# wicstas/pine

Measured on AMD Instinct MI355X. Metric: Msamples/s, higher is better.
Workload: dtype f32

## Files before the change

include/pine_gpu.h:

```cpp
#ifndef PINE_GPU_H
#define PINE_GPU_H
#include <stddef.h>
#include <stdint.h>
#ifdef __cplusplus
extern "C" {
#endif

#define PINE_GPU_ABI_VERSION 4

typedef struct pine_gpu_scene pine_gpu_scene;
typedef struct pine_gpu_plan pine_gpu_plan;

const char* pine_gpu_last_error(void);
float pine_gpu_progress(void);
int pine_gpu_abi_version(void);

void pine_gpu_mat4_identity(float out[16]);
void pine_gpu_mat4_translate(const float v[3], float out[16]);
void pine_gpu_mat4_scale(const float v[3], float out[16]);
void pine_gpu_mat4_rotate_x(float rad, float out[16]);
void pine_gpu_mat4_rotate_y(float rad, float out[16]);
void pine_gpu_mat4_rotate_z(float rad, float out[16]);
void pine_gpu_mat4_mul(const float a[16], const float b[16], float out[16]);
void pine_gpu_mat4_inverse(const float m[16], float out[16]);
// ... 145 lines not shown
  int32_t samples_per_item;
  int32_t grid_blocks;
  int32_t block_threads;
  int32_t lds_bytes;
  int32_t timed_launches;
  uint64_t walk_steps;
  float accel_build_ms;
  float upload_ms;
  int32_t accel_built_on_device;
  int32_t serial_tiles;
  int32_t specialized;
  float specialize_ms;
  uint32_t kernel_features;
  int32_t specialize_source;
  int32_t specialize_pending;
  int32_t reserved;
} pine_gpu_plan_stats;
int64_t pine_gpu_scene_specialized_source(pine_gpu_scene*, char* out, int64_t cap);
int pine_gpu_test_specialize_compile(pine_gpu_scene*, uint32_t features, int ctx, const char* arch, char* path_out, int64_t cap);
int pine_gpu_scene_build_accel_device(pine_gpu_scene*, int device);
int pine_gpu_plan_stats_get(pine_gpu_plan*, pine_gpu_plan_stats* out);
int pine_gpu_plan_check(pine_gpu_plan*);

int pine_gpu_plan_debug_sections(pine_gpu_plan*, uint64_t out[16]);
int64_t pine_gpu_plan_vertex_log(pine_gpu_plan*, float* out, int64_t capacity_floats);

int pine_gpu_plan_read_samples(pine_gpu_plan*, float* out_host, int64_t capacity_floats);

pine_gpu_plan* pine_gpu_plan_create_passes(pine_gpu_scene*, const pine_gpu_render_params*, int32_t pass_samples);
int pine_gpu_plan_pass_count(pine_gpu_plan*);
int pine_gpu_plan_pass_info(pine_gpu_plan*, int pass, int32_t out[4]);
// ... 65 lines not shown
```

pine_amd/_lib.py:

```python
import ctypes as C
import os

_HERE = os.path.dirname(os.path.abspath(__file__))
LIB_PATH = os.environ.get("PINE_GPU_LIB") or os.path.join(_HERE, "lib", "libpine_gpu.so")
TABLE_PATH = os.path.join(_HERE, "data", "bluesobol_u8.bin")

if not os.path.exists(LIB_PATH):
    raise ImportError(
        f"{LIB_PATH} not found: build the HIP extension first (python -c 'import __graft_entry__ as g; g.build()' "
        "or make -C pine_amd/csrc). pine_amd has no CPU fallback."
    )
lib = C.CDLL(LIB_PATH)

f3 = C.c_float * 3
f16 = C.c_float * 16
c_f_p = C.POINTER(C.c_float)


class RenderParams(C.Structure):
    _fields_ = [
        ("spp", C.c_int32),
        ("max_path_length", C.c_int32),
        ("device", C.c_int32),
        ("shard_rank", C.c_int32),
# ... 16 lines not shown
        ("samples_per_item", C.c_int32),
        ("grid_blocks", C.c_int32),
        ("block_threads", C.c_int32),
        ("lds_bytes", C.c_int32),
        ("timed_launches", C.c_int32),
        ("walk_steps", C.c_uint64),
        ("accel_build_ms", C.c_float),
        ("upload_ms", C.c_float),
        ("accel_built_on_device", C.c_int32),
        ("serial_tiles", C.c_int32),
        ("specialized", C.c_int32),
        ("specialize_ms", C.c_float),
        ("kernel_features", C.c_uint32),
        ("specialize_source", C.c_int32),
        ("specialize_pending", C.c_int32),
        ("reserved", C.c_int32),
    ]


FLAG_TIMING = 1
FLAG_PROGRESS = 2
FLAG_FAST = 4
FLAG_DEVICE_BVH = 8
FLAG_DEBUG_FORCE_BAIL = 0x100
FLAG_VERTEX_LOG = 0x200
FLAG_SPECIALIZE = 0x400
FLAG_SPECIALIZE_NO_BAKE = 0x800
FLAG_SPECIALIZE_ASYNC = 0x1000
FLAG_NO_SPECIALIZE = 0x2000
FLAG_ORDER_EMBREE = 0x4000
FLAG_ORDER_NEAREST = FLAG_ORDER_EMBREE
# ... 148 lines not shown
```

pine_amd/csrc/pine_kernels.hip:

```cpp
#include <hip/hip_runtime.h>

#include <climits>
#include <cmath>
#include <cstring>
#include <deque>

#include "pine_plan.h"
#include "pine_bvh_build_device.h"
#include "pine_embree_order.h"
#include "../data/rcpps_table.h"
namespace pine_gpu {

static int device_build(std::vector<BuildPrim>& prims, const std::vector<BuildTask>& roots, FlatAccel& A, int device) {
  int ndev = 0;
  if (hipGetDeviceCount(&ndev) != hipSuccess || device < 0 || device >= ndev) {
    (void)hipGetLastError();
    return -1;
  }
  if (hipSetDevice(device) != hipSuccess) return -1;
  const size_t n = prims.size();
  BuildPrim *d_prims = nullptr, *d_scratch = nullptr;
  BuildTask *d_tasks[2] = {nullptr, nullptr};
  BuildDecision* d_dec = nullptr;
  int *d_rank = nullptr, *d_perm = nullptr, *d_src = nullptr, *d_counts = nullptr;
// ... 63 lines not shown
    }
    auto by_order = [](const PineKernelVariant& a, const PineKernelVariant& b) { return a.order < b.order; };
    std::sort(queue.begin(), queue.end(), by_order);
    std::sort(mega.begin(), mega.end(), by_order);
  }
};
static const VariantTables& variant_tables() {
  static const VariantTables t;
  return t;
}
#define kVariants (variant_tables().mega)
#define kQueueVariants (variant_tables().queue)
#define kNumVariants (int(variant_tables().mega.size()))
#define kNumQueueVariants (int(variant_tables().queue.size()))

struct ResolvePass {
  int film_w, film_h, spp;
  int whole_tiles, slice_first, slice_tiles;
  int free_rows;
  int first_pass;
  int samples_so_far;
  int packed;
};
__global__ void __launch_bounds__(kBlock) resolve_kernel(WorkParams W, ResolvePass R, const float4* __restrict__ samples,
                                                        float4* __restrict__ sum, float4* __restrict__ film,
                                                        Counters* __restrict__ counters) {
  const unsigned long long t = blockIdx.x * (unsigned long long)kBlock + threadIdx.x;
  const int ltile = int(t >> 6);
  if (ltile >= W.num_local_tiles) return;
  const int p = int(t & 63);
  const int tile = film_tile_of(W, ltile);
  const int px = (tile % W.tiles_x) * kTile + (p & 7), py = (tile / W.tiles_x) * kTile + (p >> 3);
  const bool inside = px < R.film_w && py < R.film_h;
  const float4* row = nullptr;
  int rows = 0;
  bool carried = false, shown = true;
  float divisor = float(R.spp);
  if (ltile < R.whole_tiles) {
    if (ltile >= R.slice_first && ltile < R.slice_first + R.slice_tiles) {
      row = samples + (unsigned long long)(ltile - R.slice_first) * (unsigned)R.spp * 64ull + p;
      rows = R.spp;
    } else if (ltile < R.slice_first) {
      carried = true;
    } else {
      shown = false;
    }
  } else {
    row = samples + ((unsigned long long)R.slice_tiles * (unsigned)R.spp + (unsigned long long)(ltile - R.whole_tiles) * (unsigned)R.free_rows) * 64ull + p;
    rows = R.free_rows;
    carried = !R.first_pass;
    divisor = float(R.samples_so_far);
  }
  if (!inside) rows = 0;
  float4* const acc = sum && inside ? sum + (unsigned long long)ltile * 64ull + p : nullptr;
  f3 L = mk3(0.0f);
  if (carried && acc) {
    const float4 a = *acc;
    L = f3{a.x, a.y, a.z};
  }
  unsigned long long verts = 0;
  int s = 0;
  for (; s + 8 <= rows; s += 8) {
    float4 v[8];
#pragma unroll
    for (int j = 0; j < 8; j++) v[j] = row[(unsigned long long)(s + j) * 64ull];
#pragma unroll
    for (int j = 0; j < 8; j++) {
      L = L + f3{v[j].x, v[j].y, v[j].z};
      verts += (unsigned long long)v[j].w;
    }
  }
  for (; s < rows; s++) {
    const float4 v = row[(unsigned long long)s * 64ull];
    L = L + f3{v.x, v.y, v.z};
    verts += (unsigned long long)v.w;
  }
  if (inside) {
    if (acc && rows > 0) *acc = make_float4(L.x, L.y, L.z, 0.0f);
    const f3 m = L / divisor;
    const size_t out_index = R.packed ? size_t(tile / W.shard_world) * 64u + size_t(p) : size_t(py) * R.film_w + px;
    film[out_index] = shown ? make_float4(m.x, m.y, m.z, 1.0f) : make_float4(0.0f, 0.0f, 0.0f, 0.0f);
  }
  for (int off = 32; off > 0; off >>= 1) verts += __shfl_down(verts, off);
  if ((threadIdx.x & 63) == 0 && verts) atomicAdd(&counters->vertices, verts);
}

__global__ void __launch_bounds__(kBlock) unpack_film_kernel(int film_w, int film_h, int tiles_x, int total_tiles, int world,
                                                            int tiles_per_rank, const float4* __restrict__ slabs,
                                                            float4* __restrict__ film) {
  const unsigned long long t = blockIdx.x * (unsigned long long)kBlock + threadIdx.x;
  const int tile = int(t >> 6);
  if (tile >= total_tiles) return;
  const int p = int(t & 63);
  const int px = (tile % tiles_x) * kTile + (p & 7), py = (tile / tiles_x) * kTile + (p >> 3);
  if (px >= film_w || py >= film_h) return;
  const int rank = tile % world, ltile = tile / world;
  film[size_t(py) * film_w + px] = slabs[(size_t(rank) * tiles_per_rank + ltile) * 64u + p];
// ... 114 lines not shown
    if (recent.size() > kMaxLoaded) recent.pop_back();
  }
  void forget(const std::string& key) {
    std::lock_guard<std::mutex> lock(mu);
    for (auto it = recent.begin(); it != recent.end();)
      it = (*it)->key == key ? recent.erase(it) : it + 1;
  }
};

constexpr int kUnset = INT_MIN;
struct PlanKnobs {
  int specialize, lds_tris, xstage, trav_min_lanes, trav_min_trips, max_pixels, fair_period, pool_items;
  bool specialize_force, no_lds_scene, mega, no_tile_classes, no_fork, ckpt_every_launch;
  double idle_budget_s;
  int pin_kind, pin_order, lds_nodes_cap;
};
static PlanKnobs read_knobs() {
  auto num = [](const char* name) { return getenv(name) ? atoi(getenv(name)) : kUnset; };
  auto set = [](const char* name) { return getenv(name) != nullptr; };
  const char* kernel = getenv("PINE_GPU_KERNEL");
  const char* budget = getenv("PINE_GPU_IDLE_BUDGET_S");
  const int ckpt = num("PINE_GPU_CKPT_EVERY_LAUNCH");
  int pin_kind = -1, pin_order = -1;
  if (const char* pin = getenv("PINE_GPU_TEST_VARIANT")) {
    const std::string s = pin;
    const size_t colon = s.find(':');
    const std::string kind = s.substr(0, colon), digits = colon == std::string::npos ? "" : s.substr(colon + 1);
    pin_kind = kind == "queue" ? 0 : kind == "mega" ? 1 : 2;
    if (digits.empty() || digits.size() > 6 || digits.find_first_not_of("0123456789") != std::string::npos) pin_kind = 2;
    else pin_order = atoi(digits.c_str());
  }
  return PlanKnobs{num("PINE_GPU_SPECIALIZE"), num("PINE_GPU_LDS_TRIS"), num("PINE_GPU_XSTAGE"), num("PINE_GPU_TRAV_MIN_LANES"),
                   num("PINE_GPU_TRAV_MIN_TRIPS"), num("PINE_GPU_MAX_PIXELS"), num("PINE_GPU_FAIR_PERIOD"), num("PINE_GPU_POOL_ITEMS"),
                   set("PINE_GPU_SPECIALIZE_FORCE"), set("PINE_GPU_NO_LDS_SCENE"), kernel && std::string(kernel) == "mega",
                   set("PINE_GPU_NO_TILE_CLASSES"), set("PINE_GPU_NO_FORK"), ckpt != kUnset && ckpt != 0,
                   budget && atof(budget) > 0 ? atof(budget) : 30.0, pin_kind, pin_order, num("PINE_GPU_TEST_LDS_NODES")};
}

static int plan_adopt_kernel(pine_gpu_plan* p, bool compile_here);
static int plan_specialize(pine_gpu_plan* p, const FlatAccel& A, const std::vector<DShape>& shapes, const std::vector<int>& packed_prims,
                           const pine_gpu_render_params* prm, unsigned need, const PlanKnobs& K) {
  if (K.pin_kind >= 0) return 0;
  bool explicit_want = (prm->flags & PINE_GPU_FLAG_SPECIALIZE) != 0;
  bool automatic = !explicit_want && !(prm->flags & PINE_GPU_FLAG_NO_SPECIALIZE);
  if (K.specialize != kUnset) {
    if (K.specialize != 0) explicit_want = true, automatic = false;
    else explicit_want = automatic = false;
  }
  if ((!explicit_want && !automatic) || p->queue_variant < 0 || (prm->flags & (PINE_GPU_FLAG_FAST | PINE_GPU_FLAG_VERTEX_LOG))) return 0;
  const PineKernelVariant& V = kQueueVariants[p->queue_variant];
  const auto t0 = std::chrono::steady_clock::now();
// ... 874 lines not shown
  for (int j = 0; j < PP.n; j++) {
    const WorkParams Wj = pass_work(p, j);
    launch_items = std::max(launch_items, Wj.total_items);
    sample_rows = std::max(sample_rows, PP.rows(j, spp));
    ckpt_chunks = std::max(ckpt_chunks, Wj.pass_chunks);
  }
  const unsigned long long want = (launch_items + kernel.ctx - 1) / kernel.ctx;
  p->grid = int(std::min<unsigned long long>(want, (unsigned long long)prop.multiProcessorCount * blocks_per_cu));
  if (p->grid < 1) p->grid = 1;
  if (!p->serial_rng && K.pool_items == kUnset) {
    unsigned long long share = launch_items / ((unsigned long long)p->grid * 32ull);
    int claim = 512;
    while (claim < 2048 && (unsigned long long)claim * 2ull <= share) claim *= 2;
    W.pool_items = claim;
  }

  if (W.items_per_pixel > 1) {
    p->bytes_ckpt = (size_t)(W.num_local_tiles - W.serial_tiles) * ckpt_chunks * 64 * sizeof(ulonglong2);
    HIP_OK(POOL_ALLOC(p->d_ckpt, p->bytes_ckpt));
    if (PP.n > 1) {
      p->bytes_carry = (size_t)PP.free_tiles * 64 * sizeof(ulonglong2);
      HIP_OK(POOL_ALLOC(p->d_rng_carry, p->bytes_carry));
    }
  }
  if (PP.n > 1) {
    HIP_OK(POOL_ALLOC(p->d_sum, (size_t)W.num_local_tiles * 64 * sizeof(float4)));
    p->bytes_carry += (size_t)W.num_local_tiles * 64 * sizeof(float4);
  }
  p->ckpt_every_launch = K.ckpt_every_launch;
  if (!p->tile_order.empty()) {
    HIP_OK(POOL_ALLOC(p->d_tile_order, p->tile_order.size() * sizeof(int)));
    HIP_OK(hipMemcpy(p->d_tile_order, p->tile_order.data(), p->tile_order.size() * sizeof(int), hipMemcpyHostToDevice));
    W.tile_order = p->d_tile_order;
  }
  p->bytes_samples = size_t(sample_rows) * 64 * sizeof(float4);
  HIP_OK(POOL_ALLOC(p->d_samples, p->bytes_samples));
  const size_t fold_slots = size_t(p->grid) * kernel.ctx;
  HIP_OK(POOL_ALLOC(p->d_fold, size_t(prm->max_path_length) * 8 * fold_slots * sizeof(float)));
  if (kernel.queued()) {
    const size_t token_dwords = (kernel.features & F_SSS) ? size_t(p->grid) * (kernel.ctx <= 1024 ? 1024 : 2048) * kQTokenDwords : 0;
    HIP_OK(POOL_ALLOC(p->d_ctxg, (size_t(p->grid) * kernel.ctx * q_ctx_global_dwords(kernel.features) + token_dwords) * sizeof(uint32_t)));
  }
  HIP_OK(POOL_ALLOC(p->d_counters, sizeof(Counters)));
  p->timed = (prm->flags & PINE_GPU_FLAG_TIMING) != 0;
  if (p->timed)
    for (auto& slot : p->ev)
      for (auto& e : slot) HIP_OK(hipEventCreate(&e));
  return 0;
}

static int plan_build(pine_gpu_plan* p, pine_gpu_scene* scene, const pine_gpu_render_params* prm) {
  const PlanKnobs K = read_knobs();
  SceneHost& H = scene_host(scene);
  const int spp = check_params(H, prm);
  if (spp < 0) return -1;
  TableBlob tables_blob;
  if (load_tables(tables_blob)) return -1;
  int ndev = 0;
// ... 69 lines not shown
  if (j < 0 || j >= PP.n || (j != 0 && j != p->next_pass)) {
    set_error("passes run in order: pass " + std::to_string(j) + " asked for, pass " + std::to_string(p->next_pass >= PP.n ? 0 : p->next_pass) +
              (p->next_pass > 0 && p->next_pass < PP.n ? " (or 0, which starts the film afresh)" : "") + " is next; nothing was launched");
    return -1;
  }
  if (p->ao) return packed ? (set_error("an AOIntegrator plan has no packed launch"), -1) : ao_launch(p, film_dev, stream);
  HIP_OK(hipSetDevice(p->device));
  (void)hipGetLastError();
  plan_poll_background(p);
  if (j == 0) g_progress.store(0.0f);
  const int spp = p->S.spp;
  const PassPlan::Pass a = PP.pass(j, spp);
  WorkParams W = pass_work(p, j);
  const size_t film_bytes = size_t(p->film_w) * p->film_h * sizeof(float4);
  if (p->W.shard_world > 1 && !packed) HIP_OK(hipMemsetAsync(film_dev, 0, film_bytes, stream));
  HIP_OK(hipMemsetAsync(p->d_counters, 0, j == 0 ? sizeof(Counters) : sizeof(unsigned long long), stream));
  static_assert(offsetof(Counters, next_item) == 0, "the per-pass reset clears next_item");
  hipEvent_t* ev = p->ev[p->launch_count % pine_gpu_plan::kEvRing];
  if (p->timed) HIP_OK(hipEventRecord(ev[0], stream));
  const bool has_work = W.total_items > 0;
  if (has_work && p->W.items_per_pixel > 1 && PP.free_tiles > 0) {
    if (PP.n > 1 || !p->ckpt_valid || p->ckpt_every_launch) {
      const unsigned long long n = (unsigned long long)PP.free_tiles * 64ull;
      hipLaunchKernelGGL(rng_checkpoint_kernel, dim3(unsigned((n + kBlock - 1) / kBlock)), dim3(kBlock), 0, stream, W, p->film_w, p->film_h,
                         spp, p->d_ckpt, PP.free_tiles, p->d_rng_carry);
      if (PP.n == 1) {
        if (!p->ckpt_done) HIP_OK(hipEventCreateWithFlags(&p->ckpt_done, hipEventDisableTiming));
        HIP_OK(hipEventRecord(p->ckpt_done, stream));
        p->ckpt_stream = stream;
        p->ckpt_valid = true;
      }
// ... 140 lines not shown
  out->specialize_ms = p->specialize_ms;
  out->grid_blocks = p->grid;
  out->block_threads = kernel.block;
  out->lds_bytes = int(p->lds_bytes);
  out->accel_build_ms = p->accel_build_ms;
  out->accel_built_on_device = p->accel_on_device ? 1 : 0;
  out->upload_ms = p->upload_ms;
  if (p->launched) {
    HIP_OK(hipStreamSynchronize(p->last_stream));
    Counters c;
    HIP_OK(hipMemcpy(&c, p->d_counters, sizeof c, hipMemcpyDeviceToHost));
    if (plan_check_counters(c)) return -1;
    out->vertices = c.vertices;
    out->shadow_rays = c.shadow_rays;
    out->walk_steps = c.walk_steps;
    if (p->timed) {
      unsigned long long first = p->stats_read_upto;
      if (p->launch_count - first > (unsigned long long)pine_gpu_plan::kEvRing) first = p->launch_count - pine_gpu_plan::kEvRing;
      if (first == p->launch_count) first = p->launch_count - 1;
      const unsigned long long np = (unsigned long long)p->pass_plan.n;
      if (np > 1) first = p->launch_count - std::min<unsigned long long>({np, p->launch_count, (unsigned long long)pine_gpu_plan::kEvRing});
      double a = 0, b = 0, c3 = 0;
      for (unsigned long long i = first; i < p->launch_count; i++) {
        hipEvent_t* ev = p->ev[i % pine_gpu_plan::kEvRing];
        float x = 0, y = 0, z = 0;
        HIP_OK(hipEventElapsedTime(&x, ev[0], ev[1]));
        HIP_OK(hipEventElapsedTime(&y, ev[1], ev[2]));
        HIP_OK(hipEventElapsedTime(&z, ev[2], ev[3]));
        a += x, b += y, c3 += z;
      }
// ... 303 lines not shown
```

pine_amd/csrc/pine_kernels_device.h:

```cpp
#pragma once
#include <hip/hip_runtime.h>

#include <type_traits>

#include "pine_device.h"

namespace pine_gpu {

constexpr int kBlock = 256;
constexpr int kTile = 8;
#ifndef PINE_LDS_FOLD_LEVELS
#define PINE_LDS_FOLD_LEVELS 1
#endif
constexpr int kLdsFoldLevels = PINE_LDS_FOLD_LEVELS;
constexpr int kPoolItems = 128;
constexpr int kMaxDepth = 32;
constexpr unsigned kFBoxes = F_AABB | F_OBB;
constexpr unsigned kFAnalytic = F_AABB | F_OBB | F_SPHERE | F_DISK | F_CONE | F_UBER;

#ifdef PINE_PROFILE_SECTIONS
static __device__ unsigned long long g_region_lanes[16], g_region_hits[16];
#ifndef PINE_PROFILE_REGIONS
#define REGION(id)
#else
// ... 141 lines not shown
  int debug_force_bail;
  int trav_min_lanes, trav_min_trips;
  int fair_period;
  int pick_spins;
  int pool_items;
  int max_pixels;
  int fork_sealed;
  unsigned long long* progress;
  float* vertex_log;
  int pass_first_chunk;
  int pass_chunks;
  unsigned pass_chunks_magic;
  int pass_row_stride;
  int free_tile_base;
  int pass_first_serial_tile;
};
constexpr int kVertexLogFloats = 16;
__device__ __forceinline__ void post_progress(const WorkParams& W, unsigned long long claimed, unsigned shift) {
  if (W.progress && ((claimed >> shift) & 15ull) == 0ull)
    __hip_atomic_store(W.progress, claimed, __ATOMIC_RELAXED, __HIP_MEMORY_SCOPE_SYSTEM);
}

struct TravLog {
  unsigned* words;
  int n, cap;
  __device__ __forceinline__ void put(unsigned w) {
    if (n < cap) words[n] = w;
    n++;
  }
};
// ... 455 lines not shown
  const int px = (tile % W.tiles_x) * kTile + (p & 7), py = (tile / W.tiles_x) * kTile + (p >> 3);
  DRng g = rng_seed(hash_pixel(px, py, 0));
  if (carry && W.pass_first_chunk != 0) {
    const ulonglong2 c = carry[t];
    g = DRng{c.x, c.y};
  }
  for (int c = 0; c < W.pass_chunks; c++) {
    const unsigned long long item = ((unsigned long long)ptile * W.pass_chunks + c) * 64ull + p;
    ckpt[item] = make_ulonglong2(g.s0, g.s1);
    for (int i = 0; i < 4 * W.samples_per_item; i++) rng_next64(g);
  }
  if (carry) carry[t] = make_ulonglong2(g.s0, g.s1);
  (void)film_w, (void)film_h, (void)spp;
}

struct Counters {
  unsigned long long next_item;
  unsigned long long vertices;
  unsigned long long shadow_rays;
  unsigned long long bail_count;
  unsigned long long bail_code, bail_a, bail_b;
  unsigned long long walk_steps;
  unsigned long long section_cycles[16];
  unsigned long long t_start, t_pool_dry, t_end;
#ifdef PINE_PROFILE_SECTIONS
  unsigned long long wg_t[1024][4];
#endif
};



__device__ __forceinline__ f3 material_le(const DMaterial* m, f3 n, f3 wo) {
  if (m->kind != MAT_EMISSIVE) return mk3(0.0f);
  if (dot(wo, n) < 0.0f) return mk3(0.0f);
  return ld3(m->color);
}

// ... 316 lines not shown
```

pine_amd/csrc/pine_queue_kernel.h:

```cpp
#pragma once


namespace pine_gpu {

#ifndef PINE_QBLOCK
#define PINE_QBLOCK 1024
#endif
constexpr int kQBlock = PINE_QBLOCK;
#ifndef PINE_QCTX
#define PINE_QCTX 1536
#endif
constexpr int kQFields = 12;
enum : int { QS_S = 0, QS_T = 1, QS_W = 2, QS_XS = 3, QS_XC = 4 };
constexpr int q_num_stage_queues(unsigned F) { return ((F & F_LDS_TOP) && (F & F_XSTAGE)) ? 5 : (F & F_SSS) ? 3 : 2; }
constexpr int q_num_queues(unsigned F) { return q_num_stage_queues(F) + ((F & F_SSS) ? 2 : 0); }
enum : int { CF_OX, CF_OY, CF_OZ, CF_DX, CF_DY, CF_DZ, CF_TMAX, CF_ST, CF_PXY, CF_SBASE, CF_GEOM, CF_PRIM };
constexpr unsigned kStFresh = 0xffffffffu;
enum : int { QC_HEAD = 0, QC_TAIL = 8, QC_BUSY = 16, QC_LOCK = 17, QC_EXHAUSTED = 18, QC_PNEXT = 20, QC_PEND = 22, QC_ABORT = 24, QC_PIXELS = 25, QC_WORDS = 32 };
constexpr int kQTokenDwords = 8;
constexpr unsigned kQSpinLimit = 1u << 22;
constexpr int kQWinDwords = 5;

template <int CTX, int NQ = 2, bool ALIAS = false>
struct QLayout {
  static constexpr int ctx = CTX;
  static constexpr int ring = CTX <= 1024 ? 1024 : 2048;
  static constexpr int off_ctl = 0;
  static constexpr int off_ring = off_ctl + QC_WORDS;
  static constexpr int off_state = off_ring + NQ * ring;
  static constexpr int off_sobol = off_state + kQFields * CTX;
  static constexpr int off_win = off_sobol + kLdsSamplerDims * 256 / 4;
  static constexpr int off_stack = ALIAS ? off_win : off_win + kQWinDwords * kQBlock;
  static constexpr size_t fixed_bytes = size_t(off_stack) * 4;
// ... 250 lines not shown
      SEC_MARK(6);
      finish_hit(id, hit, ray.tmax, geom, prim, st, to_shade, to_term);
    }
  };

  unsigned shadow_count = 0, walk_count = 0;
  unsigned spins = 0;
  unsigned pick_no = 0;
  unsigned idle_polls = 0;
  auto bail = [&](unsigned code, unsigned a, unsigned b) {
    __atomic_store_n(&qctl[QC_ABORT], 1u, __ATOMIC_RELAXED);
    atomicAdd(&counters->bail_count, 1ull);
    counters->bail_code = code;
    counters->bail_a = a;
    counters->bail_b = b;
  };

  auto wake_free = [&](unsigned count) {
    if constexpr (kFork) {
      const unsigned fh = __builtin_amdgcn_readfirstlane(lds_load(&qctl[QC_HEAD + QS_F]));
      const unsigned favail = __builtin_amdgcn_readfirstlane(lds_load(&qctl[QC_TAIL + QS_F])) - fh;
      if (favail != 0u && count != 0u) {
        const unsigned want = favail < count ? favail : count;
        unsigned got = 0;
        if (lane == 0) got = atomicCAS(&qctl[QC_HEAD + QS_F], fh, fh + want) == fh ? 1u : 0u;
        if (__builtin_amdgcn_readfirstlane(got)) {
          int fid = -1;
          if (lane < want) {
            unsigned* slot = &ring[QS_F * kQRing + ((fh + lane) & (kQRing - 1))];
            unsigned v, tries = 0;
// ... 617 lines not shown
          cstu[CF_ST * kQCtx + id] = st.v;
        }
      }
      SEC_MARK(13);
      __builtin_amdgcn_fence(__ATOMIC_RELEASE, "workgroup");
      push2(to_shade, false, id);
      push_w(to_walk, id);
    } else {
      bool need_item = false, have_path = false;
      bool to_shade2 = false, to_term2 = false, to_xc2 = false;
      bool to_free = false;
      bool fresh_rng = false;
      bool free_item = false;
      bool wake_more = false;
      DRng item_rng{0, 0};
      unsigned pxy = 0, sample_base = 0;
      int s_next = 0;
      uint4 rng_words = make_uint4(0, 0, 0, 0);
      if (valid) {
        REGION(13);
        rng_words = *reinterpret_cast<const uint4*>(ctx_global(id));
        const PackedState st{cstu[CF_ST * kQCtx + id]};
        if (st.v == kStFresh) {
          need_item = true;
        } else {
          const int pv_length = st.length();
          const int geom = int(cstu[CF_GEOM * kQCtx + id]);
          f3 Lo = mk3(0.0f);
          bool lp_valid = false;
          float lp = 0.0f;
// ... 38 lines not shown
            }
          };
          int level = pv_length - 1;
          for (; level >= 0; level--) {
            const float4* q = fold_entry(id, level);
            fold_step(q[0], q[1], level);
          }
          const int s_now = st.s_cur();
          sample_base = cstu[CF_SBASE * kQCtx + id];
          pxy = cstu[CF_PXY * kQCtx + id];
          samples[size_t(sample_base) + size_t(s_now) * 64u] = make_float4(Li.x, Li.y, Li.z, float(pv_length + 1));
          s_next = s_now + 1;
          const bool item_done = kFork ? chain_ends_at(s_next) : closes_item(W.samples_per_item, s_next);
          if ((kFork && st.sealed()) || item_done) need_item = true;
          else have_path = true;
          if constexpr (kFork)
            if (!st.sealed() && chain_ends_at(s_next)) {
              const unsigned before = atomicSub(&qctl[QC_PIXELS], 1u);
              (void)before;
#ifdef PINE_PROFILE_SECTIONS
              if (before == 1u && blockIdx.x < 1024) counters->wg_t[blockIdx.x][0] = wall_clock64();
#endif
            }
        }
      }
      SEC_MARK(7);
      for (unsigned rounds = 0;; rounds++) {
        const unsigned long long m = __ballot(need_item);
        if (m == 0) break;
        if (rounds > 4096u) {
          if (lane == 0) bail(4, unsigned(m), unsigned(m >> 32));
          need_item = false;
          break;
        }
        const unsigned want_all = __popcll(m);
        unsigned want = want_all;
        unsigned long long base = 0;
        unsigned got = 0;
        unsigned kbase = 0, kgot = 0;
        unsigned want_free = 0;
        unsigned free_items_left = 0;
        if (lane == 0) {
          unsigned tries = 0;
          while (atomicCAS(&qctl[QC_LOCK], 0u, 1u) != 0u) {
            if (++tries > kQSpinLimit) {
              bail(3, 0, 0);
              break;
            }
            __builtin_amdgcn_s_sleep(1);
          }
          __builtin_amdgcn_fence(__ATOMIC_ACQUIRE, "workgroup");
          if constexpr (kFork) {
            kbase = lds_load(&qctl[QC_HEAD + QS_K]);
            const unsigned kavail = lds_load(&qctl[QC_TAIL + QS_K]) - kbase;
            kgot = want < kavail ? want : kavail;
            __atomic_store_n(&qctl[QC_HEAD + QS_K], kbase + kgot, __ATOMIC_RELAXED);
            want -= kgot;
            want_free = want;
            const unsigned inflight = lds_load(&qctl[QC_PIXELS]);
            const unsigned room = inflight < unsigned(kW(max_pixels)) ? unsigned(kW(max_pixels)) - inflight : 0u;
            if (want > room) want = room;
          }
          unsigned long long nx = (unsigned long long)lds_load(&qctl[QC_PNEXT]) | ((unsigned long long)lds_load(&qctl[QC_PNEXT + 1]) << 32);
          unsigned long long en = (unsigned long long)lds_load(&qctl[QC_PEND]) | ((unsigned long long)lds_load(&qctl[QC_PEND + 1]) << 32);
          if (want != 0u && nx == en && lds_load(&qctl[QC_EXHAUSTED]) == 0u) {
            const unsigned long long b = atomicAdd(&counters->next_item, (unsigned long long)kW(pool_items));
            if (b >= kW(total_items)) {
#ifdef PINE_PROFILE_SECTIONS
              atomicCAS(&counters->t_pool_dry, 0ull, wall_clock64());
              if (blockIdx.x < 1024) counters->wg_t[blockIdx.x][1] = wall_clock64();
#endif
              __atomic_store_n(&qctl[QC_EXHAUSTED], 1u, __ATOMIC_RELAXED);
            } else {
              post_progress(W, b, 9);
#ifdef PINE_PROFILE_SECTIONS
              if (blockIdx.x < 1024) {
                if (b < (unsigned long long)W.serial_tiles * 64ull) atomicAdd(&counters->wg_t[blockIdx.x][3], 64ull);
              }
#endif
              nx = b;
              en = b + kW(pool_items) < kW(total_items) ? b + kW(pool_items) : kW(total_items);
            }
          }
          const unsigned long long avail = en - nx;
          if constexpr (kFork) {
            if (W.serial_tiles > 0 && nx >= (unsigned long long)W.serial_tiles * 64ull) want = want_free;
          }
          got = want < avail ? want : unsigned(avail);
          if constexpr (kFork) {
            if (!(W.serial_tiles > 0 && nx >= (unsigned long long)W.serial_tiles * 64ull)) atomicAdd(&qctl[QC_PIXELS], got);
            else if (avail > got) free_items_left = 1u;
          }
          base = nx;
          nx += got;
          __atomic_store_n(&qctl[QC_PNEXT], unsigned(nx), __ATOMIC_RELAXED);
          __atomic_store_n(&qctl[QC_PNEXT + 1], unsigned(nx >> 32), __ATOMIC_RELAXED);
          __atomic_store_n(&qctl[QC_PEND], unsigned(en), __ATOMIC_RELAXED);
          __atomic_store_n(&qctl[QC_PEND + 1], unsigned(en >> 32), __ATOMIC_RELAXED);
          __builtin_amdgcn_fence(__ATOMIC_RELEASE, "workgroup");
          __atomic_store_n(&qctl[QC_LOCK], 0u, __ATOMIC_RELAXED);
        }
        base = __shfl(base, 0);
        got = __shfl(got, 0);
        if constexpr (kFork) {
          kbase = __shfl(kbase, 0);
          kgot = __shfl(kgot, 0);
          wake_more |= __shfl(free_items_left, 0) != 0u;
        }
        if (got == 0 && kgot == 0) {
          if constexpr (kFork) to_free = need_item;
          need_item = false;
          break;
        }
        unsigned rank = __popcll(m & ((1ull << lane) - 1ull));
        if (kFork && need_item && rank < kgot) {
          const unsigned pos = (kbase + rank) & (kQRing - 1);
          unsigned* flag = &ring[QS_K * kQRing + pos];
          unsigned tries = 0;
// ... 4 lines not shown
            }
            __builtin_amdgcn_s_sleep(1);
          }
          __builtin_amdgcn_fence(__ATOMIC_ACQUIRE, "workgroup");
          const uint4* tok = reinterpret_cast<const uint4*>(token_slot(pos));
          const uint4 g = tok[0], b = tok[1];
          need_item = false;
          have_path = true;
          pxy = b.x;
          sample_base = b.y;
          s_next = int(b.z);
          item_rng = DRng{uint64_t(g.x) | (uint64_t(g.y) << 32), uint64_t(g.z) | (uint64_t(g.w) << 32)};
          fresh_rng = true;
        }
        rank -= kgot;
        if (need_item && rank < got) {
          const unsigned long long item = base + rank;
          WorkParams Wl;
          kload(kWOffset, &Wl);
          const ItemInfo itf = decode_item(Wl, kS(cam.W), kS(cam.H), kS(spp), item);
          if (itf.valid) {
            need_item = false;
            have_path = true;
            pxy = unsigned(itf.px) | (unsigned(itf.py) << 16);
            sample_base = unsigned(itf.sample_base);
            s_next = itf.chunk * W.samples_per_item;
            DRng g;
            if (itf.serial || W.items_per_pixel == 1) {
              g = rng_seed(hash_pixel(itf.px, itf.py, 0));
            } else {
              const ulonglong2 c = ckpt[itf.ckpt_index];
              g = DRng{c.x, c.y};
            }
            item_rng = g;
            fresh_rng = true;
            if constexpr (kFork) free_item = W.serial_tiles > 0 && !itf.serial;
          } else {
            if constexpr (kFork)
              if (!(W.serial_tiles > 0 && !itf.serial)) atomicSub(&qctl[QC_PIXELS], 1u);
          }
        }
      }
      if constexpr (kFork)
        if (to_free) cstu[CF_ST * kQCtx + id] = kStFresh;
      SEC_MARK(8);
      if (valid && have_path) {
        uint4* cg4 = reinterpret_cast<uint4*>(ctx_global(id));
        DRng g = item_rng;
        if (!fresh_rng)
          g = DRng{uint64_t(rng_words.x) | (uint64_t(rng_words.y) << 32), uint64_t(rng_words.z) | (uint64_t(rng_words.w) << 32)};
        const int px = int(pxy & 0xffffu), py = int(pxy >> 16);
        const DCamera cam = kS(cam);
        const DRay r = camera_sample(cam, px, py, g);
        cg4[0] = make_uint4(uint32_t(g.s0), uint32_t(g.s0 >> 32), uint32_t(g.s1), uint32_t(g.s1 >> 32));
        if constexpr (kBigDim) ctx_global(id)[6] = S.tables.kind == 2 ? 2u : 0u;
        PackedState st{0};
// ... 2 lines not shown
          if (free_item) st.set_sealed();
        if constexpr (F & F_SOBOL)
          if (S.tables.kind == 2) st.set_dim(2);
        cstu[CF_PXY * kQCtx + id] = pxy;
        cstu[CF_SBASE * kQCtx + id] = sample_base;
        extend(id, r.o, r.d, r.tmax, st, to_shade2, to_term2, to_xc2);
      }
      SEC_MARK(9);
      __builtin_amdgcn_fence(__ATOMIC_RELEASE, "workgroup");
      push2(to_shade2, to_term2, id);
      if constexpr (kX) push_q(QS_XC, to_xc2, id);
      if constexpr (kFork) {
        push_q(QS_F, to_free, id);
        if (wake_more) wake_free(64u);
      }
    }
    if (lane == 0) atomicSub(&qctl[QC_BUSY], 1u);
  }

#ifdef PINE_PROFILE_SECTIONS
  if (tid == 0) atomicMax(&counters->t_end, wall_clock64());
  if (tid == 0 && blockIdx.x < 1024) counters->wg_t[blockIdx.x][2] = wall_clock64();
#endif
  SEC_FLUSH();
  unsigned long long sc = shadow_count;
  for (int off = 32; off > 0; off >>= 1) sc += __shfl_down(sc, off);
  if (lane == 0) atomicAdd(&counters->shadow_rays, sc);
  if constexpr (F & F_SSS) {
    unsigned long long wc = walk_count;
    for (int off = 32; off > 0; off >>= 1) wc += __shfl_down(wc, off);
// ... 13 lines not shown
```

Before: 10150.

## Resolve owned tiles inside the queued path-tracing kernel as they finish

Work claims for the first tiles are resized to whole tiles, and each workgroup tracks per-tile completion counts in LDS slots. When a tile's last sample finishes, the workgroup sums its sample rows and writes the film pixels itself, then marks the tile done so the separate resolve kernel skips it. The aim is to overlap the resolve pass with tracing and cut the trailing resolve's memory traffic. In exchange it adds LDS scanning and atomics on the hot loop, plus a tile-granular claim pattern that may hurt load balance.

Result: faster. 10380 (median of 6 runs) (+2.3%).

```diff
diff --git a/include/pine_gpu.h b/include/pine_gpu.h
--- a/include/pine_gpu.h
+++ b/include/pine_gpu.h
@@ -183,7 +183,7 @@
   uint32_t kernel_features;
   int32_t specialize_source;
   int32_t specialize_pending;
-  int32_t reserved;
+  int32_t tiles_in_kernel;
 } pine_gpu_plan_stats;
 int64_t pine_gpu_scene_specialized_source(pine_gpu_scene*, char* out, int64_t cap);
 int pine_gpu_test_specialize_compile(pine_gpu_scene*, uint32_t features, int ctx, const char* arch, char* path_out, int64_t cap);
diff --git a/pine_amd/_lib.py b/pine_amd/_lib.py
--- a/pine_amd/_lib.py
+++ b/pine_amd/_lib.py
@@ -54,7 +54,7 @@
         ("kernel_features", C.c_uint32),
         ("specialize_source", C.c_int32),
         ("specialize_pending", C.c_int32),
-        ("reserved", C.c_int32),
+        ("tiles_in_kernel", C.c_int32),
     ]
 
 
diff --git a/pine_amd/csrc/pine_kernels.hip b/pine_amd/csrc/pine_kernels.hip
--- a/pine_amd/csrc/pine_kernels.hip
+++ b/pine_amd/csrc/pine_kernels.hip
@@ -101,73 +101,14 @@
 #define kNumVariants (int(variant_tables().mega.size()))
 #define kNumQueueVariants (int(variant_tables().queue.size()))
 
-struct ResolvePass {
-  int film_w, film_h, spp;
-  int whole_tiles, slice_first, slice_tiles;
-  int free_rows;
-  int first_pass;
-  int samples_so_far;
-  int packed;
-};
 __global__ void __launch_bounds__(kBlock) resolve_kernel(WorkParams W, ResolvePass R, const float4* __restrict__ samples,
                                                         float4* __restrict__ sum, float4* __restrict__ film,
                                                         Counters* __restrict__ counters) {
   const unsigned long long t = blockIdx.x * (unsigned long long)kBlock + threadIdx.x;
   const int ltile = int(t >> 6);
   if (ltile >= W.num_local_tiles) return;
-  const int p = int(t & 63);
-  const int tile = film_tile_of(W, ltile);
-  const int px = (tile % W.tiles_x) * kTile + (p & 7), py = (tile / W.tiles_x) * kTile + (p >> 3);
-  const bool inside = px < R.film_w && py < R.film_h;
-  const float4* row = nullptr;
-  int rows = 0;
-  bool carried = false, shown = true;
-  float divisor = float(R.spp);
-  if (ltile < R.whole_tiles) {
-    if (ltile >= R.slice_first && ltile < R.slice_first + R.slice_tiles) {
-      row = samples + (unsigned long long)(ltile - R.slice_first) * (unsigned)R.spp * 64ull + p;
-      rows = R.spp;
-    } else if (ltile < R.slice_first) {
-      carried = true;
-    } else {
-      shown = false;
-    }
-  } else {
-    row = samples + ((unsigned long long)R.slice_tiles * (unsigned)R.spp + (unsigned long long)(ltile - R.whole_tiles) * (unsigned)R.free_rows) * 64ull + p;
-    rows = R.free_rows;
-    carried = !R.first_pass;
-    divisor = float(R.samples_so_far);
-  }
-  if (!inside) rows = 0;
-  float4* const acc = sum && inside ? sum + (unsigned long long)ltile * 64ull + p : nullptr;
-  f3 L = mk3(0.0f);
-  if (carried && acc) {
-    const float4 a = *acc;
-    L = f3{a.x, a.y, a.z};
-  }
-  unsigned long long verts = 0;
-  int s = 0;
-  for (; s + 8 <= rows; s += 8) {
-    float4 v[8];
-#pragma unroll
-    for (int j = 0; j < 8; j++) v[j] = row[(unsigned long long)(s + j) * 64ull];
-#pragma unroll
-    for (int j = 0; j < 8; j++) {
-      L = L + f3{v[j].x, v[j].y, v[j].z};
-      verts += (unsigned long long)v[j].w;
-    }
-  }
-  for (; s < rows; s++) {
-    const float4 v = row[(unsigned long long)s * 64ull];
-    L = L + f3{v.x, v.y, v.z};
-    verts += (unsigned long long)v.w;
-  }
-  if (inside) {
-    if (acc && rows > 0) *acc = make_float4(L.x, L.y, L.z, 0.0f);
-    const f3 m = L / divisor;
-    const size_t out_index = R.packed ? size_t(tile / W.shard_world) * 64u + size_t(p) : size_t(py) * R.film_w + px;
-    film[out_index] = shown ? make_float4(m.x, m.y, m.z, 1.0f) : make_float4(0.0f, 0.0f, 0.0f, 0.0f);
-  }
+  if (W.tile_done && W.tile_done[ltile]) return;
+  unsigned long long verts = resolve_tile<8>(W, R, samples, sum, film, ltile, int(t & 63));
   for (int off = 32; off > 0; off >>= 1) verts += __shfl_down(verts, off);
   if ((threadIdx.x & 63) == 0 && verts) atomicAdd(&counters->vertices, verts);
 }
@@ -312,6 +253,7 @@
   bool specialize_force, no_lds_scene, mega, no_tile_classes, no_fork, ckpt_every_launch;
   double idle_budget_s;
   int pin_kind, pin_order, lds_nodes_cap;
+  int owned_tiles, tile_slots;
 };
 static PlanKnobs read_knobs() {
   auto num = [](const char* name) { return getenv(name) ? atoi(getenv(name)) : kUnset; };
@@ -332,7 +274,8 @@
                    num("PINE_GPU_TRAV_MIN_TRIPS"), num("PINE_GPU_MAX_PIXELS"), num("PINE_GPU_FAIR_PERIOD"), num("PINE_GPU_POOL_ITEMS"),
                    set("PINE_GPU_SPECIALIZE_FORCE"), set("PINE_GPU_NO_LDS_SCENE"), kernel && std::string(kernel) == "mega",
                    set("PINE_GPU_NO_TILE_CLASSES"), set("PINE_GPU_NO_FORK"), ckpt != kUnset && ckpt != 0,
-                   budget && atof(budget) > 0 ? atof(budget) : 30.0, pin_kind, pin_order, num("PINE_GPU_TEST_LDS_NODES")};
+                   budget && atof(budget) > 0 ? atof(budget) : 30.0, pin_kind, pin_order, num("PINE_GPU_TEST_LDS_NODES"),
+                   num("PINE_GPU_OWNED_TILES"), num("PINE_GPU_TEST_TILE_SLOTS")};
 }
 
 static int plan_adopt_kernel(pine_gpu_plan* p, bool compile_here);
@@ -1237,6 +1180,18 @@
     while (claim < 2048 && (unsigned long long)claim * 2ull <= share) claim *= 2;
     W.pool_items = claim;
   }
+  W.owned_tiles = 0;
+  W.pool_items_log2 = 0;
+  while ((1 << W.pool_items_log2) < W.pool_items) W.pool_items_log2++;
+  W.tile_slots = K.tile_slots != kUnset ? std::max(0, std::min(K.tile_slots, kQTileSlots)) : kQTileSlots;
+  const bool can_own = kernel.queued() && !(kernel.features & F_SSS) && !p->fast && PP.n == 1 && W.serial_tiles == 0 && p->tile_order.empty() &&
+                       W.free_tile_base == 0 && (1 << W.pool_items_log2) == W.pool_items && W.total_items > 0;
+  if (can_own) {
+    const long long tile_items = 64ll * W.pass_chunks;
+    long long owned = tile_items >= std::max(W.pool_items, kernel.ctx) ? (long long)W.num_local_tiles - 2ll * p->grid : 0;
+    if (K.owned_tiles != kUnset) owned = K.owned_tiles;
+    W.owned_tiles = int(std::max(0ll, std::min<long long>(owned, W.num_local_tiles)));
+  }
 
   if (W.items_per_pixel > 1) {
     p->bytes_ckpt = (size_t)(W.num_local_tiles - W.serial_tiles) * ckpt_chunks * 64 * sizeof(ulonglong2);
@@ -1264,7 +1219,8 @@
     const size_t token_dwords = (kernel.features & F_SSS) ? size_t(p->grid) * (kernel.ctx <= 1024 ? 1024 : 2048) * kQTokenDwords : 0;
     HIP_OK(POOL_ALLOC(p->d_ctxg, (size_t(p->grid) * kernel.ctx * q_ctx_global_dwords(kernel.features) + token_dwords) * sizeof(uint32_t)));
   }
-  HIP_OK(POOL_ALLOC(p->d_counters, sizeof(Counters)));
+  HIP_OK(POOL_ALLOC(p->d_counters, sizeof(Counters) + (W.owned_tiles > 0 ? size_t(W.num_local_tiles) * sizeof(unsigned) : 0)));
+  W.tile_done = W.owned_tiles > 0 ? reinterpret_cast<unsigned*>(p->d_counters + 1) : nullptr;
   p->timed = (prm->flags & PINE_GPU_FLAG_TIMING) != 0;
   if (p->timed)
     for (auto& slot : p->ev)
@@ -1364,7 +1320,10 @@
   WorkParams W = pass_work(p, j);
   const size_t film_bytes = size_t(p->film_w) * p->film_h * sizeof(float4);
   if (p->W.shard_world > 1 && !packed) HIP_OK(hipMemsetAsync(film_dev, 0, film_bytes, stream));
-  HIP_OK(hipMemsetAsync(p->d_counters, 0, j == 0 ? sizeof(Counters) : sizeof(unsigned long long), stream));
+  const size_t done_bytes = p->W.tile_done ? size_t(p->W.num_local_tiles) * sizeof(unsigned) : 0;
+  HIP_OK(hipMemsetAsync(p->d_counters, 0, j == 0 ? sizeof(Counters) + done_bytes : sizeof(unsigned long long), stream));
+  W.film = (float4*)film_dev;
+  W.film_packed = packed ? 1 : 0;
   static_assert(offsetof(Counters, next_item) == 0, "the per-pass reset clears next_item");
   hipEvent_t* ev = p->ev[p->launch_count % pine_gpu_plan::kEvRing];
   if (p->timed) HIP_OK(hipEventRecord(ev[0], stream));
@@ -1535,6 +1494,7 @@
     out->vertices = c.vertices;
     out->shadow_rays = c.shadow_rays;
     out->walk_steps = c.walk_steps;
+    out->tiles_in_kernel = int32_t(c.tiles_summed);
     if (p->timed) {
       unsigned long long first = p->stats_read_upto;
       if (p->launch_count - first > (unsigned long long)pine_gpu_plan::kEvRing) first = p->launch_count - pine_gpu_plan::kEvRing;
diff --git a/pine_amd/csrc/pine_kernels_device.h b/pine_amd/csrc/pine_kernels_device.h
--- a/pine_amd/csrc/pine_kernels_device.h
+++ b/pine_amd/csrc/pine_kernels_device.h
@@ -179,6 +179,12 @@
   int pass_row_stride;
   int free_tile_base;
   int pass_first_serial_tile;
+  int owned_tiles;
+  int pool_items_log2;
+  int tile_slots;
+  int film_packed;
+  float4* film;
+  unsigned* tile_done;
 };
 constexpr int kVertexLogFloats = 16;
 __device__ __forceinline__ void post_progress(const WorkParams& W, unsigned long long claimed, unsigned shift) {
@@ -664,6 +670,72 @@
   (void)film_w, (void)film_h, (void)spp;
 }
 
+struct ResolvePass {
+  int film_w, film_h, spp;
+  int whole_tiles, slice_first, slice_tiles;
+  int free_rows;
+  int first_pass;
+  int samples_so_far;
+  int packed;
+};
+template <int ROWS>
+__device__ __forceinline__ unsigned long long resolve_tile(const WorkParams& W, const ResolvePass& R, const float4* samples, float4* sum,
+                                                           float4* film, int ltile, int p) {
+  const int tile = film_tile_of(W, ltile);
+  const int px = (tile % W.tiles_x) * kTile + (p & 7), py = (tile / W.tiles_x) * kTile + (p >> 3);
+  const bool inside = px < R.film_w && py < R.film_h;
+  const float4* row = nullptr;
+  int rows = 0;
+  bool carried = false, shown = true;
+  float divisor = float(R.spp);
+  if (ltile < R.whole_tiles) {
+    if (ltile >= R.slice_first && ltile < R.slice_first + R.slice_tiles) {
+      row = samples + (unsigned long long)(ltile - R.slice_first) * (unsigned)R.spp * 64ull + p;
+      rows = R.spp;
+    } else if (ltile < R.slice_first) {
+      carried = true;
+    } else {
+      shown = false;
+    }
+  } else {
+    row = samples + ((unsigned long long)R.slice_tiles * (unsigned)R.spp + (unsigned long long)(ltile - R.whole_tiles) * (unsigned)R.free_rows) * 64ull + p;
+    rows = R.free_rows;
+    carried = !R.first_pass;
+    divisor = float(R.samples_so_far);
+  }
+  if (!inside) rows = 0;
+  float4* const acc = sum && inside ? sum + (unsigned long long)ltile * 64ull + p : nullptr;
+  f3 L = mk3(0.0f);
+  if (carried && acc) {
+    const float4 a = *acc;
+    L = f3{a.x, a.y, a.z};
+  }
+  unsigned long long verts = 0;
+  int s = 0;
+  for (; s + ROWS <= rows; s += ROWS) {
+    float4 v[ROWS];
+#pragma unroll
+    for (int j = 0; j < ROWS; j++) v[j] = row[(unsigned long long)(s + j) * 64ull];
+#pragma unroll
+    for (int j = 0; j < ROWS; j++) {
+      L = L + f3{v[j].x, v[j].y, v[j].z};
+      verts += (unsigned long long)v[j].w;
+    }
+  }
+  for (; s < rows; s++) {
+    const float4 v = row[(unsigned long long)s * 64ull];
+    L = L + f3{v.x, v.y, v.z};
+    verts += (unsigned long long)v.w;
+  }
+  if (inside) {
+    if (acc && rows > 0) *acc = make_float4(L.x, L.y, L.z, 0.0f);
+    const f3 m = L / divisor;
+    const size_t out_index = R.packed ? size_t(tile / W.shard_world) * 64u + size_t(p) : size_t(py) * R.film_w + px;
+    film[out_index] = shown ? make_float4(m.x, m.y, m.z, 1.0f) : make_float4(0.0f, 0.0f, 0.0f, 0.0f);
+  }
+  return verts;
+}
+
 struct Counters {
   unsigned long long next_item;
   unsigned long long vertices;
@@ -671,6 +743,7 @@
   unsigned long long bail_count;
   unsigned long long bail_code, bail_a, bail_b;
   unsigned long long walk_steps;
+  unsigned long long tiles_summed;
   unsigned long long section_cycles[16];
   unsigned long long t_start, t_pool_dry, t_end;
 #ifdef PINE_PROFILE_SECTIONS
diff --git a/pine_amd/csrc/pine_queue_kernel.h b/pine_amd/csrc/pine_queue_kernel.h
--- a/pine_amd/csrc/pine_queue_kernel.h
+++ b/pine_amd/csrc/pine_queue_kernel.h
@@ -16,7 +16,9 @@
 constexpr int q_num_queues(unsigned F) { return q_num_stage_queues(F) + ((F & F_SSS) ? 2 : 0); }
 enum : int { CF_OX, CF_OY, CF_OZ, CF_DX, CF_DY, CF_DZ, CF_TMAX, CF_ST, CF_PXY, CF_SBASE, CF_GEOM, CF_PRIM };
 constexpr unsigned kStFresh = 0xffffffffu;
-enum : int { QC_HEAD = 0, QC_TAIL = 8, QC_BUSY = 16, QC_LOCK = 17, QC_EXHAUSTED = 18, QC_PNEXT = 20, QC_PEND = 22, QC_ABORT = 24, QC_PIXELS = 25, QC_WORDS = 32 };
+enum : int { QC_HEAD = 0, QC_TAIL = 8, QC_BUSY = 16, QC_LOCK = 17, QC_EXHAUSTED = 18, QC_PNEXT = 20, QC_PEND = 22, QC_ABORT = 24, QC_PIXELS = 25, QC_PSLOT = 26,
+             QC_TILE = 32, QC_TILE_LEFT = 36, QC_WORDS = 40 };
+constexpr int kQTileSlots = 4;
 constexpr int kQTokenDwords = 8;
 constexpr unsigned kQSpinLimit = 1u << 22;
 constexpr int kQWinDwords = 5;
@@ -297,6 +299,37 @@
     counters->bail_code = code;
     counters->bail_a = a;
     counters->bail_b = b;
+  };
+
+  auto tile_sum = [&](unsigned slot) {
+    __builtin_amdgcn_fence(__ATOMIC_ACQUIRE, "workgroup");
+    SEC_MARK(10);
+    const unsigned key = __builtin_amdgcn_readfirstlane(lds_load(&qctl[QC_TILE + slot]));
+    WorkParams Wl;
+    kload(kWOffset, &Wl);
+    const int spp = kS(spp);
+    const int tile = int(key >> 19) * Wl.tiles_x + int((key & 0xffffu) >> 3);
+    const int ltile = tile / Wl.shard_world;
+    const ResolvePass R{kS(cam.W), kS(cam.H), spp, 0, 0, 0, spp, 1, spp, Wl.film_packed};
+    unsigned long long verts = resolve_tile<16>(Wl, R, samples, nullptr, Wl.film, ltile, int(lane));
+    for (int off = 32; off > 0; off >>= 1) verts += __shfl_down(verts, off);
+    if (lane == 0) {
+      if (verts) atomicAdd(&counters->vertices, verts);
+      atomicAdd(&counters->tiles_summed, 1ull);
+      Wl.tile_done[ltile] = 1u;
+      __atomic_store_n(&qctl[QC_TILE + slot], 0u, __ATOMIC_RELAXED);
+    }
+    SEC_MARK(14);
+  };
+  auto tile_count_off = [&](unsigned slot, bool flag) -> unsigned {
+    const unsigned long long m = __ballot(flag);
+    if (m == 0) return 0u;
+    unsigned last = 0;
+    if (lane == 0) {
+      const unsigned n = unsigned(__popcll(m));
+      last = atomicSub(&qctl[QC_TILE_LEFT + slot], n) == n ? 1u : 0u;
+    }
+    return __builtin_amdgcn_readfirstlane(last) << slot;
   };
 
   auto wake_free = [&](unsigned count) {
@@ -944,6 +977,8 @@
       bool free_item = false;
       bool wake_more = false;
       DRng item_rng{0, 0};
+      unsigned done_slot = 0;
+      unsigned sum_slots = 0;
       unsigned pxy = 0, sample_base = 0;
       int s_next = 0;
       uint4 rng_words = make_uint4(0, 0, 0, 0);
@@ -1012,6 +1047,13 @@
           const bool item_done = kFork ? chain_ends_at(s_next) : closes_item(W.samples_per_item, s_next);
           if ((kFork && st.sealed()) || item_done) need_item = true;
           else have_path = true;
+          if constexpr (!kFork)
+            if (item_done) {
+              const unsigned key = (pxy & 0xfff8fff8u) | 1u;
+#pragma unroll
+              for (int k = 0; k < kQTileSlots; k++)
+                if (lds_load(&qctl[QC_TILE + k]) == key) done_slot = unsigned(k + 1);
+            }
           if constexpr (kFork)
             if (!st.sealed() && chain_ends_at(s_next)) {
               const unsigned before = atomicSub(&qctl[QC_PIXELS], 1u);
@@ -1037,6 +1079,7 @@
         unsigned got = 0;
         unsigned kbase = 0, kgot = 0;
         unsigned want_free = 0;
+        unsigned pslot = 0;
         unsigned free_items_left = 0;
         if (lane == 0) {
           unsigned tries = 0;
@@ -1062,7 +1105,19 @@
           unsigned long long nx = (unsigned long long)lds_load(&qctl[QC_PNEXT]) | ((unsigned long long)lds_load(&qctl[QC_PNEXT + 1]) << 32);
           unsigned long long en = (unsigned long long)lds_load(&qctl[QC_PEND]) | ((unsigned long long)lds_load(&qctl[QC_PEND + 1]) << 32);
           if (want != 0u && nx == en && lds_load(&qctl[QC_EXHAUSTED]) == 0u) {
-            const unsigned long long b = atomicAdd(&counters->next_item, (unsigned long long)kW(pool_items));
+            unsigned long long b = atomicAdd(&counters->next_item, (unsigned long long)kW(pool_items));
+            unsigned long long claim_items = (unsigned long long)kW(pool_items);
+            bool owned = false;
+            if constexpr (!kFork) {
+              const unsigned long long owned_tiles = (unsigned long long)unsigned(kW(owned_tiles));
+              if (owned_tiles != 0ull) {
+                const unsigned long long c = b >> unsigned(kW(pool_items_log2));
+                const unsigned long long tile_items = 64ull * unsigned(kW(pass_chunks));
+                owned = c < owned_tiles;
+                if (owned) b = c * tile_items, claim_items = tile_items;
+                else b = (c - owned_tiles) * claim_items + owned_tiles * tile_items;
+              }
+            }
             if (b >= kW(total_items)) {
 #ifdef PINE_PROFILE_SECTIONS
               atomicCAS(&counters->t_pool_dry, 0ull, wall_clock64());
@@ -1077,9 +1132,28 @@
               }
 #endif
               nx = b;
-              en = b + kW(pool_items) < kW(total_items) ? b + kW(pool_items) : kW(total_items);
-            }
-          }
+              en = b + claim_items < kW(total_items) ? b + claim_items : kW(total_items);
+              if constexpr (!kFork) {
+                unsigned slot1 = 0;
+                if (owned) {
+                  const unsigned ltile = unsigned(b / claim_items);
+                  const unsigned tile = ltile * unsigned(kW(shard_world)) + unsigned(kW(shard_rank));
+                  const unsigned tiles_x = unsigned(kW(tiles_x));
+                  const unsigned key = (((tile % tiles_x) * kTile) | (((tile / tiles_x) * kTile) << 16)) | 1u;
+                  const unsigned slots = unsigned(kW(tile_slots));
+                  for (unsigned k = 0; k < unsigned(kQTileSlots) && k < slots; k++)
+                    if (lds_load(&qctl[QC_TILE + k]) == 0u) {
+                      __atomic_store_n(&qctl[QC_TILE_LEFT + k], unsigned(claim_items), __ATOMIC_RELAXED);
+                      __atomic_store_n(&qctl[QC_TILE + k], key, __ATOMIC_RELAXED);
+                      slot1 = k + 1;
+                      break;
+                    }
+                }
+                __atomic_store_n(&qctl[QC_PSLOT], slot1, __ATOMIC_RELAXED);
+              }
+            }
+          }
+          if constexpr (!kFork) pslot = lds_load(&qctl[QC_PSLOT]);
           const unsigned long long avail = en - nx;
           if constexpr (kFork) {
             if (W.serial_tiles > 0 && nx >= (unsigned long long)W.serial_tiles * 64ull) want = want_free;
@@ -1100,6 +1174,7 @@
         }
         base = __shfl(base, 0);
         got = __shfl(got, 0);
+        if constexpr (!kFork) pslot = __builtin_amdgcn_readfirstlane(pslot);
         if constexpr (kFork) {
           kbase = __shfl(kbase, 0);
           kgot = __shfl(kgot, 0);
@@ -1134,6 +1209,7 @@
           fresh_rng = true;
         }
         rank -= kgot;
+        bool off_film = false;
         if (need_item && rank < got) {
           const unsigned long long item = base + rank;
           WorkParams Wl;
@@ -1156,10 +1232,13 @@
             fresh_rng = true;
             if constexpr (kFork) free_item = W.serial_tiles > 0 && !itf.serial;
           } else {
+            off_film = true;
             if constexpr (kFork)
               if (!(W.serial_tiles > 0 && !itf.serial)) atomicSub(&qctl[QC_PIXELS], 1u);
           }
         }
+        if constexpr (!kFork)
+          if (pslot != 0u) sum_slots |= tile_count_off(pslot - 1u, off_film);
       }
       if constexpr (kFork)
         if (to_free) cstu[CF_ST * kQCtx + id] = kStFresh;
@@ -1192,6 +1271,17 @@
         push_q(QS_F, to_free, id);
         if (wake_more) wake_free(64u);
       }
+      if constexpr (!kFork) {
+        if (__ballot(done_slot != 0u) != 0ull) {
+#pragma unroll
+          for (unsigned k = 0; k < unsigned(kQTileSlots); k++) sum_slots |= tile_count_off(k, done_slot == k + 1u);
+        }
+        while (sum_slots != 0u) {
+          const unsigned k = unsigned(__builtin_ctz(sum_slots));
+          sum_slots &= sum_slots - 1u;
+          tile_sum(k);
+        }
+      }
     }
     if (lane == 0) atomicSub(&qctl[QC_BUSY], 1u);
   }
```
